# ChangUk/RecommenderSystems

Measured on AMD Instinct MI355X. Metric: RWR seeds/sec + achieved HBM GB/s on 100M-edge bipartite graph, 1/2/4/8 GPUs, higher is better.
Workload: dtype f64

## Files before the change

### include/rwr.h

```cpp
#ifndef RWR_H
#define RWR_H

#include <stdint.h>

#ifdef __cplusplus
extern "C" {
#endif

#define RWR_VERSION_STRING "0.4.0"

enum {
    RWR_OK            = 0,
    RWR_E_INVALID     = 1,
    RWR_E_RANGE       = 2,
    RWR_E_NO_DEVICE   = 3,
    RWR_E_HIP         = 4,
    RWR_E_NOMEM       = 5,
    RWR_E_CAPACITY    = 6,
    RWR_E_UNSUPPORTED = 7
};

enum { RWR_NODE_UNDEFINED = 0, RWR_NODE_USER = 1, RWR_NODE_ITEM = 2, RWR_NODE_ETC = 3 };
enum { RWR_EDGE_UNDEFINED = 0, RWR_EDGE_LIKE = 1, RWR_EDGE_FRIENDSHIP = 2, RWR_EDGE_FOLLOW = 3,
       RWR_EDGE_MENTION = 4, RWR_EDGE_AUTHORSHIP = 5, RWR_EDGE_PURCHASE = 6, RWR_EDGE_ETC = 7 };
// ... 12 lines not shown
    int32_t tile_group;
    int32_t profile;
    int64_t workspace_bytes;
    int32_t seed_row_kernel;
    int32_t reserved0;
} rwr_opts;

typedef struct rwr_stats {
    int32_t struct_size;
    int32_t n;
    int64_t nnz_raw;
    int64_t nnz;
    int32_t uniform;
    int32_t tile_seeds;
    int32_t tile_group;
    int32_t mode;
    double  build_ms;
    double  spmm_ms;
    int64_t spmm_launches;
    int64_t spmm_seed_steps;
    double  chain_ms;
    int64_t chain_launches;
    double  rank_ms;
    double  iterate_wall_ms;
    double  total_wall_ms;
    int64_t seeds_done;
    int64_t chain_redo_blocks;
    double  spmm_dense_ms;
    int64_t spmm_dense_launches;
    int64_t spmm_dense_seed_steps;
    int32_t uniform_path;
    int32_t reserved1;
    int64_t frontier_list_launches;
} rwr_stats;


const char *rwr_version(void);
int32_t rwr_device_count(void);
const char *rwr_last_error(void);

int32_t rwr_graph_create(int32_t n, const int64_t *node_id, const uint8_t *node_type,
                         const int64_t *rowptr , const int32_t *dst, const uint8_t *etype,
                         const double *w, const rwr_opts *opts , rwr_graph **out);
int32_t rwr_graph_destroy(rwr_graph *g);
int32_t rwr_graph_update_links(rwr_graph *g, int64_t count, const int64_t *link_index,
                               const uint8_t *etype , const double *w );
int32_t rwr_graph_append_links(rwr_graph *g, int64_t count, const int32_t *src, const int32_t *dst,
                               const uint8_t *etype, const double *w,
                               int64_t *new_index_out );
int32_t rwr_graph_size(const rwr_graph *g, int32_t *n, int64_t *nnz_raw, int64_t *nnz_explicit);
int32_t rwr_graph_get_normalized(rwr_graph *g, double *w_out , uint8_t *dangling_out );

int32_t rwr_recommend(rwr_graph *g, int32_t seed, float d, int32_t n_iter, int32_t top_n,
                      int64_t *out_id, double *out_score, int64_t *inout_count);

int32_t rwr_recommend_eval(rwr_graph *g, int32_t seed, float d, int32_t n_iter, const int64_t *test_ids,
                           int64_t n_test, int64_t *n_hits, double *sum_precision, int64_t *list_len);

int32_t rwr_recommend_eval_batch(rwr_graph *g, const int32_t *seeds, int32_t K, float d, int32_t n_iter,
                                 const int64_t *test_ptr, const int64_t *test_ids, int64_t *n_hits,
                                 double *sum_precision, int64_t *list_len);

typedef struct rwr_graph_desc {
    int32_t n_nodes;
    int32_t reserved0;
    const int64_t *node_id;
// ... 43 lines not shown
```

### recommendersystems_amd/_lib.py

```python
from __future__ import annotations

import ctypes as C
import os

_HERE = os.path.dirname(os.path.abspath(__file__))
LIB_PATH = os.path.join(_HERE, "librwr.so")

RWR_OK, RWR_E_INVALID, RWR_E_RANGE, RWR_E_NO_DEVICE, RWR_E_HIP, RWR_E_NOMEM, RWR_E_CAPACITY, RWR_E_UNSUPPORTED = range(8)
RWR_MODE_EXACT = 0
RWR_RUN_ITERATIONS, RWR_RUN_THRESHOLD, RWR_RUN_DEFAULT_THRESHOLD = 0, 1, 2

EXPORTS = [
    "rwr_version", "rwr_device_count", "rwr_last_error",
    "rwr_graph_create", "rwr_graph_update_links", "rwr_graph_append_links", "rwr_graph_destroy", "rwr_graph_size", "rwr_graph_get_normalized",
    "rwr_recommend", "rwr_recommend_eval", "rwr_recommend_eval_batch", "rwr_eval_graphs", "rwr_recommend_batch", "rwr_model_run", "rwr_model_deliver",
    "rwr_model_run_restart", "rwr_model_deliver_restart", "rwr_model_run_batch", "rwr_model_run_restart_batch",
    "rwr_part_begin", "rwr_part_step", "rwr_part_local_step", "rwr_part_finish_step", "rwr_part_rank",
    "rwr_get_stats", "rwr_reset_stats",
]


class rwr_opts(C.Structure):
    _fields_ = [("struct_size", C.c_int32), ("device", C.c_int32), ("mode", C.c_int32),
                ("tile_seeds", C.c_int32), ("tile_group", C.c_int32), ("profile", C.c_int32),
                ("workspace_bytes", C.c_int64), ("seed_row_kernel", C.c_int32), ("reserved0", C.c_int32)]


class rwr_graph_desc(C.Structure):
    _fields_ = [("n_nodes", C.c_int32), ("reserved0", C.c_int32), ("node_id", C.POINTER(C.c_int64)),
                ("node_type", C.POINTER(C.c_uint8)), ("rowptr", C.POINTER(C.c_int64)), ("dst", C.POINTER(C.c_int32)),
                ("etype", C.POINTER(C.c_uint8)), ("w", C.POINTER(C.c_double))]


class rwr_stats(C.Structure):
    _fields_ = [("struct_size", C.c_int32), ("n", C.c_int32), ("nnz_raw", C.c_int64), ("nnz", C.c_int64),
                ("uniform", C.c_int32), ("tile_seeds", C.c_int32), ("tile_group", C.c_int32), ("mode", C.c_int32),
                ("build_ms", C.c_double), ("spmm_ms", C.c_double), ("spmm_launches", C.c_int64),
                ("spmm_seed_steps", C.c_int64), ("chain_ms", C.c_double), ("chain_launches", C.c_int64),
                ("rank_ms", C.c_double), ("iterate_wall_ms", C.c_double), ("total_wall_ms", C.c_double),
                ("seeds_done", C.c_int64), ("chain_redo_blocks", C.c_int64),
                ("spmm_dense_ms", C.c_double), ("spmm_dense_launches", C.c_int64), ("spmm_dense_seed_steps", C.c_int64),
                ("uniform_path", C.c_int32), ("reserved1", C.c_int32), ("frontier_list_launches", C.c_int64)]


class RwrError(RuntimeError):
    def __init__(self, status: int, message: str):
        super().__init__(f"librwr status {status}: {message}")
        self.status = status


_lib = None


def load():
    global _lib
    if _lib is not None:
        return _lib
    if not os.path.exists(LIB_PATH):
        raise ImportError(f"{LIB_PATH} not found: build it with `python -c 'import __graft_entry__ as g; g.build()'` "
                          "(hipcc --offload-arch=gfx950); there is no CPU fallback")
    lib = C.CDLL(LIB_PATH)
    p = C.POINTER
    lib.rwr_version.restype = C.c_char_p
    lib.rwr_last_error.restype = C.c_char_p
    lib.rwr_device_count.restype = C.c_int32
    lib.rwr_graph_create.restype = C.c_int32
    lib.rwr_graph_create.argtypes = [C.c_int32, p(C.c_int64), p(C.c_uint8), p(C.c_int64), p(C.c_int32),
                                     p(C.c_uint8), p(C.c_double), p(rwr_opts), p(C.c_void_p)]
    lib.rwr_graph_update_links.restype = C.c_int32
    lib.rwr_graph_update_links.argtypes = [C.c_void_p, C.c_int64, p(C.c_int64), p(C.c_uint8), p(C.c_double)]
    lib.rwr_graph_append_links.restype = C.c_int32
    lib.rwr_graph_append_links.argtypes = [C.c_void_p, C.c_int64, p(C.c_int32), p(C.c_int32), p(C.c_uint8), p(C.c_double),
                                           p(C.c_int64)]
    lib.rwr_graph_destroy.restype = C.c_int32
    lib.rwr_graph_destroy.argtypes = [C.c_void_p]
# ... 58 lines not shown
```

### recommendersystems_amd/csrc/api.hip

```cpp
#include <stdarg.h>
#include <algorithm>
#include <cmath>
#include <mutex>
#include <vector>
#include <stdlib.h>
#include <string.h>

#include "engine.h"

namespace rwr {

static thread_local char g_err[512] = "";

void set_error(const char *fmt, ...)
{
    va_list ap;
    va_start(ap, fmt);
    vsnprintf(g_err, sizeof(g_err), fmt, ap);
    va_end(ap);
}

static int usable_devices()
{
    int n = 0;
// ... 896 lines not shown
    if (!g || !dev_y || !dev_r) { set_error("rwr_part_finish_step: NULL argument"); return RWR_E_INVALID; }
    RWR_BIND(g);
    return part_finish_step(g, (double *)dev_y, (const double *)dev_r);
}

int32_t rwr_part_rank(rwr_graph *g, void *dev_x, int32_t top_n, int64_t *ids, double *scores, int32_t *counts)
{
    g_err[0] = 0;
    if (!g || !dev_x || !ids || !scores || !counts) { set_error("rwr_part_rank: NULL argument"); return RWR_E_INVALID; }
    RWR_BIND(g);
    return part_rank(g, (double *)dev_x, top_n, ids, scores, counts);
}

int32_t rwr_get_stats(rwr_graph *g, rwr_stats *out)
{
    if (!g || !out) { set_error("rwr_get_stats: NULL argument"); return RWR_E_INVALID; }
    size_t sz = out->struct_size > 0 ? (size_t)out->struct_size : sizeof(rwr_stats);
    if (sz > sizeof(rwr_stats)) sz = sizeof(rwr_stats);
    rwr_stats s = g->stats;
    s.struct_size = (int32_t)sz;
    memcpy(out, &s, sz);
    return RWR_OK;
}

int32_t rwr_reset_stats(rwr_graph *g)
{
    if (!g) { set_error("rwr_reset_stats: NULL argument"); return RWR_E_INVALID; }
    rwr_stats &s = g->stats;
    s.spmm_ms = s.chain_ms = s.rank_ms = s.iterate_wall_ms = s.total_wall_ms = 0;
    s.spmm_launches = s.spmm_seed_steps = s.chain_launches = s.seeds_done = s.chain_redo_blocks = 0;
    s.spmm_dense_ms = 0;
    s.spmm_dense_launches = s.spmm_dense_seed_steps = 0;
    s.frontier_list_launches = 0;
    return RWR_OK;
}

}
```

### recommendersystems_amd/csrc/iterate.h

```cpp
#pragma once
#include "engine.h"
#include "step_plan.h"

namespace rwr {

struct SpmmArgs {
    const double *X = nullptr;
    double *Y = nullptr;
    const int32_t *seeds = nullptr;
    double c1 = 0.0;
    bool skip_seed_row = false;
    const uint32_t *nz_in = nullptr;
    uint32_t *nz_out = nullptr;
    const uint32_t *act = nullptr;
    const double *Zin = nullptr;
    double *Zout = nullptr;
    bool hub_scan = false;
    RowSource rows{};
};
void launch_spmm(rwr_graph *g, int G, int tg, const SpmmArgs &a, hipStream_t s);
void launch_init_seeds(rwr_graph *g, int G, int tg, double *X, const int32_t *seeds, uint32_t *nz, double *Z, double c1,
                       hipStream_t s);
void launch_make_z(int64_t elems, int G, const double *X, double *Z, const double *w_src, double c1, hipStream_t s);
void launch_make_z_nz(rwr_graph *g, int32_t lo, int32_t hi, int G, const double *X, double *Zs, double c1, uint32_t *nz,
// ... 1 lines not shown
void launch_mark_active(rwr_graph *g, int G, int tg, const uint32_t *nz, uint32_t *act, const int32_t *seeds, int32_t *fl_rows,
                        int32_t *fl_cnt, hipStream_t s);

struct Profile {
    const bool on;
    std::vector<hipEvent_t> pool, spmm, chain, rank, iter;
    size_t used = 0;
    std::vector<uint8_t> dense;
    explicit Profile(const rwr_graph *g) : on(g->opts.profile != 0) {}
    ~Profile() { for (auto e : pool) (void)hipEventDestroy(e); }
    int32_t record(hipEvent_t &e, hipStream_t s);
    int32_t end(std::vector<hipEvent_t> &stage, hipEvent_t a, hipStream_t s);
    void reset() { spmm.clear(); chain.clear(); rank.clear(); iter.clear(); dense.clear(); used = 0; }
    int32_t fold(rwr_graph *g);
};

struct GroupIter {
    rwr_graph *g;
    int G, tg;
    const int32_t *d_seeds;
    const int64_t *d_evoff;
    double c1;
    double *X, *Y;
    double *Zc = nullptr, *Zn = nullptr;
    uint32_t *nz_cur = nullptr, *nz_oth = nullptr;
    PlanConfig cfg;
    int64_t it = 0;
    int64_t dense_steps = 0;

    GroupIter(rwr_graph *g_, int G_, int tg_, const int32_t *seeds, const int64_t *evoff, double d)
        : g(g_), G(G_), tg(tg_), d_seeds(seeds), d_evoff(evoff), c1(1 - d) ,
          X(g_->X.p), Y(g_->Y.p), Zc(g_->vf ? g_->Z0.p : nullptr), Zn(g_->vf ? g_->Z1.p : nullptr) {}

    int32_t init(bool fresh = true, bool ranks_nonneg = true, bool ranking_only = false);
    int32_t step(const StepPlan &p, Profile &prof);
};

int32_t iterate_group(rwr_graph *g, int G, int tg, const int32_t *d_seeds, const int64_t *d_evoff, const int32_t *h_seeds,
                      double d, int64_t T, Profile &prof, double **final_X, int64_t *dense_steps);

int resolve_G(const rwr_graph *g, int32_t K);
int32_t ensure_workspace(rwr_graph *g, int G, int32_t K, int *TG_out, int extra_mats = 0);
int32_t upload_seed_slots(rwr_graph *g, const int32_t *seeds, int32_t K, int G, std::vector<int32_t> *slot_k_out,
                          std::vector<int32_t> *slot_seed_out = nullptr);

}
```

### recommendersystems_amd/csrc/iterate.hip

```cpp
#include "iterate.h"

#include <climits>
#include <cstdlib>
#include <type_traits>

namespace rwr {

template <int G, bool VF>
__global__ __launch_bounds__(256) void k_spmm(int32_t n, const int64_t *__restrict__ in_ptr,
                                              const int32_t *__restrict__ in_src,
                                              const double *__restrict__ in_w,
                                              const int32_t *__restrict__ row_order, int32_t nrows,
                                              const double *__restrict__ X, double *__restrict__ Y,
                                              const int32_t *__restrict__ seeds, double c1, int skip_seed_row,
                                              const double *__restrict__ w_src, double *__restrict__ Zout)
{
    constexpr int RPW = WAVE / G;
    constexpr int U = 4;
    const int tile = blockIdx.y;
    const size_t toff = (size_t)tile * (size_t)n * G;
    X += toff;
    Y += toff;
    if (VF && Zout) Zout += toff;
    const int lane = threadIdx.x & (WAVE - 1);
// ... 32 lines not shown
        }
        for (; p < e; ++p) {
            if (VF) {
                acc += X[(size_t)in_src[p] * G + k];
            } else {
                double rw = c1 * X[(size_t)in_src[p] * G + k];
                acc += rw * in_w[p];
            }
        }
        if (j >= 0 && j != my_seed) {
            Y[(size_t)j * G + k] = acc;
            if (VF && Zout) { const double rw = c1 * acc; Zout[(size_t)j * G + k] = rw * w_src[j]; }
        }
    }
}

template <int G, int CH, bool CHECK, bool WRITE, bool VF>
__device__ __forceinline__ void spmm_chunked_body(int32_t n, const int64_t *__restrict__ in_ptr,
                                                  const int32_t *__restrict__ in_src,
                                                  const double *__restrict__ in_w,
                                                  const int32_t *__restrict__ row_order, int32_t nrows,
                                                  const double *__restrict__ X, double *__restrict__ Y,
                                                  const int32_t *__restrict__ seeds, double c1,
                                                  int skip_seed_row, const uint32_t *__restrict__ nz_in,
                                                  uint32_t *__restrict__ nz_out,
                                                  const uint32_t *__restrict__ act,
                                                  const double *__restrict__ w_src, double *__restrict__ Zout)
{
    static_assert(G >= 8 && G <= 64, "chunked SpMM needs 8 <= G <= 64");
    constexpr int RPW = WAVE / G;
    const int tile = blockIdx.y;
    const size_t toff = (size_t)tile * (size_t)n * G;
    X += toff;
    Y += toff;
    if (VF && Zout) Zout += toff;
    const size_t nzw = ((size_t)n + 31) / 32;
    if (CHECK) nz_in += (size_t)tile * nzw;
    if (WRITE) nz_out += (size_t)tile * nzw;
    if (CHECK && act) act += (size_t)tile * nzw;
    const int lane = threadIdx.x & (WAVE - 1);
    const int sub = lane / G, k = lane % G;
    const int gbase = (lane - k) << 2;
    const int32_t my_seed = skip_seed_row ? seeds[tile * G + k] : -1;
    const int wpb = blockDim.x / WAVE;
    const int64_t nwaves = (int64_t)gridDim.x * wpb;
    for (int64_t rb = ((int64_t)blockIdx.x * wpb + threadIdx.x / WAVE) * RPW; rb < nrows; rb += nwaves * RPW) {
        const int64_t r = rb + sub;
        int32_t j = -1;
        int64_t p = 0, e = 0;
        if (r < nrows) {
            j = row_order[r];
            p = in_ptr[j];
            e = in_ptr[j + 1];
            if (CHECK && act && !((act[(uint32_t)j >> 5] >> (j & 31)) & 1u)) e = p;
        }
        double acc = 0.0;
        while (__any(p < e)) {
            const int64_t left = e - p;
            const int cnt = left > CH ? CH : (left > 0 ? (int)left : 0);
            int32_t my_idx = 0;
            double my_w = 0.0;
            if (k < cnt) {
                my_idx = in_src[p + k];
                if (!VF) my_w = in_w[p + k];
                if (CHECK) {
                    const uint32_t wd = nz_in[(uint32_t)my_idx >> 5];
                    if (!((wd >> (my_idx & 31)) & 1u)) my_idx |= (int32_t)0x80000000;
// ... 23 lines not shown
                                acc += rw * __hiloint2double(hi, lo);
                            }
                        }
                    }
                    p += cnt;
                    continue;
                }
            }
            double xv[CH], wv[CH];
#pragma unroll
            for (int t = 0; t < CH; ++t) {
                const int idx = __builtin_amdgcn_ds_bpermute(gbase + (t << 2), my_idx);
                if (!VF) {
                    const int lo = __builtin_amdgcn_ds_bpermute(gbase + (t << 2), wlo);
                    const int hi = __builtin_amdgcn_ds_bpermute(gbase + (t << 2), whi);
                    wv[t] = __hiloint2double(hi, lo);
                }
                xv[t] = (t < cnt && idx >= 0) ? X[(size_t)idx * G + k] : 0.0;
            }
#pragma unroll
            for (int t = 0; t < CH; ++t) {
                if (t < cnt) {
                    if (VF) {
                        acc += xv[t];
                    } else {
                        double rw = c1 * xv[t];
                        acc += rw * wv[t];
                    }
                }
            }
            p += cnt;
        }
        if (j >= 0 && j != my_seed) {
            Y[(size_t)j * G + k] = acc;
            if (VF && Zout) { const double rw = c1 * acc; Zout[(size_t)j * G + k] = rw * w_src[j]; }
        }
        if (WRITE) {
            const unsigned long long nzb = __ballot(acc != 0.0);
            const unsigned long long gmask = (G == 64) ? ~0ull : (((1ull << (G & 63)) - 1ull) << (sub * G));
            if (k == 0 && j >= 0 && (nzb & gmask)) atomicOr(&nz_out[(uint32_t)j >> 5], 1u << (j & 31));
        }
    }
}

template <int G, int CH, bool CHECK, bool WRITE, bool VF, bool LIST>
__global__ __launch_bounds__(256) void k_spmm_chunked(int32_t n, const int64_t *__restrict__ in_ptr,
                                                      const int32_t *__restrict__ in_src,
                                                      const double *__restrict__ in_w,
                                                      const int32_t *__restrict__ row_order, int32_t nrows,
                                                      const double *__restrict__ X, double *__restrict__ Y,
                                                      const int32_t *__restrict__ seeds, double c1,
                                                      int skip_seed_row, const uint32_t *__restrict__ nz_in,
                                                      uint32_t *__restrict__ nz_out,
                                                      const uint32_t *__restrict__ act,
                                                      const double *__restrict__ w_src, double *__restrict__ Zout)
{
    spmm_chunked_body<G, CH, CHECK, WRITE, VF>(n, in_ptr, in_src, in_w, row_order, nrows, X, Y, seeds, c1, skip_seed_row,
                                               nz_in, nz_out, act, w_src, Zout);
}

template <int G, int CH, bool VF>
__global__ __launch_bounds__(256) void k_spmm_frontier(int32_t n, const int64_t *__restrict__ in_ptr,
                                                       const int32_t *__restrict__ in_src,
                                                       const double *__restrict__ in_w,
                                                       const int32_t *__restrict__ fl_rows,
                                                       const int32_t *__restrict__ fl_cnt,
                                                       const double *__restrict__ X, double *__restrict__ Y,
// ... 185 lines not shown
    double acc = 0.0;
    for (size_t w0 = 0; w0 < nzw; w0 += WAVE) {
        const uint32_t word = (w0 + lane < nzw) ? bits[w0 + lane] : 0u;
        unsigned long long mask = __ballot(word != 0u);
        while (mask) {
            const int l = __builtin_ctzll(mask);
            mask &= mask - 1;
            uint32_t wv = (uint32_t)__builtin_amdgcn_readlane((int)word, l);
            while (wv) {
                const int b = __builtin_ctz(wv);
                wv &= wv - 1;
                const int32_t i = (int32_t)((w0 + l) * 32 + b);
                if (consumer && s >= 0) {
                    while (p < e && in_src[p] < i) ++p;
                    while (p < e && in_src[p] == i) { acc += termp[p]; ++p; }
                    const double xi = x[(size_t)i * G + k];
                    const double rw = c1 * xi;
                    acc += dangling[i] ? xi : (xi - rw);
                }
            }
        }
    }
    if (consumer && s >= 0) {
        Y[(size_t)tile * (size_t)n * G + (size_t)s * G + k] = acc;
        if (nz_out && acc != 0.0)
            atomicOr(&nz_out[(size_t)tile * nzw + ((uint32_t)s >> 5)], 1u << (s & 31));
    }
}

constexpr int CH3_NSW = 6;
constexpr int CH3_NST = CH3_NSW * WAVE;
constexpr int CH3_LPT = 16;
constexpr int CH3_CE = CH3_NST * CH3_LPT;
template <int G>
__global__ __launch_bounds__(WAVE + CH3_NST) void k_seed_chain_roles(
    int32_t n, const int64_t *__restrict__ in_ptr, const int32_t *__restrict__ in_src,
    const uint8_t *__restrict__ dangling, const double *__restrict__ X, double *__restrict__ Y,
    const int32_t *__restrict__ seeds, double c1, const int64_t *__restrict__ evoff,
    const double *__restrict__ evterm, uint32_t *__restrict__ nz_out, unsigned int *__restrict__ gate)
{
    if (threadIdx.x == 0 && gate) __hip_atomic_fetch_add(gate, 1u, __ATOMIC_RELAXED, __HIP_MEMORY_SCOPE_AGENT);
    constexpr int CR = CH3_CE / G;
    static_assert(CR % 32 == 0, "chunk rows must be a multiple of 32");
    extern __shared__ double rr[];
    const int tile = blockIdx.x;
    const double *x = X + (size_t)tile * (size_t)n * G;
    const int tid = threadIdx.x;
    const int64_t total = (int64_t)n * G;
    const int nchunks = (int)((total + CH3_CE - 1) / CH3_CE);

    if (tid >= WAVE) {
        const int st = tid - WAVE;
        double rega[CH3_LPT], regb[CH3_LPT];
        uint8_t dga[CH3_LPT], dgb[CH3_LPT];
#define CH3_LOAD(R, D, C)                                                       \
    {                                                                           \
        const int64_t base__ = (int64_t)(C) * CH3_CE;                           \
        _Pragma("unroll") for (int u = 0; u < CH3_LPT; ++u) {                   \
            int64_t el = base__ + (int64_t)u * CH3_NST + st;                    \
            el = el < total ? el : total - 1;                                   \
            R[u] = x[el];                                                       \
            D[u] = dangling[el / G];                                            \
        }                                                                       \
    }
#define CH3_STAGE(R, D, C)                                                                              \
    {                                                                                                   \
        const int64_t base__ = (int64_t)(C) * CH3_CE;                                                   \
        double *buf__ = rr + (size_t)((C) & 1) * CH3_CE;                                                \
        _Pragma("unroll") for (int u = 0; u < CH3_LPT; ++u) {                                           \
            const int off = u * CH3_NST + st;                                                           \
            const double xv = (base__ + off < total) ? R[u] : 0.0;   \
            const double rw = c1 * xv;                                                                  \
            buf__[off] = D[u] ? xv : (xv - rw);                                                         \
        }                                                                                               \
    }
        CH3_LOAD(rega, dga, 0)
        if (nchunks > 1) CH3_LOAD(regb, dgb, 1)
        for (int c = 0; c < nchunks; c += 2) {
            CH3_STAGE(rega, dga, c)
            if (c + 2 < nchunks) CH3_LOAD(rega, dga, c + 2)
            __builtin_amdgcn_fence(__ATOMIC_RELEASE, "workgroup", "local");
            __builtin_amdgcn_s_barrier();
            if (c + 1 < nchunks) {
                CH3_STAGE(regb, dgb, c + 1)
                if (c + 3 < nchunks) CH3_LOAD(regb, dgb, c + 3)
                __builtin_amdgcn_fence(__ATOMIC_RELEASE, "workgroup", "local");
                __builtin_amdgcn_s_barrier();
            }
        }
#undef CH3_LOAD
#undef CH3_STAGE
        return;
    }

    const bool consumer = tid < G;
    const int k = tid % G;
    int32_t s = -1;
    int64_t p = 0, e = 0;
    const int32_t *srcp = in_src;
    const double *termp = evterm;
    int32_t nxt = INT_MAX, raw_s = INT_MAX;
    double tcur = 0.0, raw_t = 0.0;
    bool has2 = false;
    if (consumer) {
        s = seeds[tile * G + k];
        if (s >= 0) {
            p = in_ptr[s];
            e = in_ptr[s + 1];
            termp = evterm + evoff[tile * G + k] - p;
            if (p < e) { nxt = srcp[p]; tcur = termp[p]; ++p; }
            if (p < e) { raw_s = srcp[p]; raw_t = termp[p]; has2 = true; ++p; }
        }
    }
    double acc = 0.0;
    __builtin_amdgcn_s_setprio(3);
    for (int c = 0; c < nchunks; ++c) {
        __builtin_amdgcn_s_barrier();
        __builtin_amdgcn_fence(__ATOMIC_ACQUIRE, "workgroup", "local");
// ... 91 lines not shown
    const int64_t j = ((int64_t)lo & ~(int64_t)63) + (int64_t)blockIdx.x * blockDim.x + threadIdx.x;
    bool any = false;
    if (j >= lo && j < hi) {
        const double w = w_src[j];
        const size_t at = (size_t)(j - lo) * G;
        for (int k = 0; k < G; ++k) {
            const double xv = X[(size_t)j * G + k];
            const double rw = c1 * xv;
            Zs[at + k] = rw * w;
            any = any || xv != 0.0;
        }
    }
    const unsigned long long m = __ballot(any);
    const int lane = threadIdx.x & (WAVE - 1);
    if (lane == 0 && (uint32_t)m) nz[(uint64_t)j >> 5] = (uint32_t)m;
    if (lane == 32 && (uint32_t)(m >> 32)) nz[(uint64_t)j >> 5] = (uint32_t)(m >> 32);
}


static PlanInput read_plan_knobs()
{
    PlanInput v;
    const char *e;
    if ((e = getenv("RWR_SPMM"))) v.spmm = atoi(e);
    if ((e = RWR_TUNE_ENV("RWR_NZ_ITERS"))) v.nz_iters = atoi(e);
    if ((e = getenv("RWR_ACT_ITERS"))) v.act_iters = atoi(e);
    if ((e = RWR_TUNE_ENV("RWR_ACT_MIN_N"))) v.act_min_n = atol(e);
    if ((e = getenv("RWR_FRONTIER_LIST"))) v.frontier_list = atoi(e);
    if ((e = getenv("RWR_CHAIN"))) v.chain = atoi(e);
    if ((e = RWR_TUNE_ENV("RWR_SCAN_WORK"))) v.scan_work = atof(e);
    if ((e = RWR_TUNE_ENV("RWR_SCAN_SIDE"))) v.scan_side = atoi(e);
    if ((e = RWR_TUNE_ENV("RWR_GATE"))) v.gate = atoi(e);
    if ((e = getenv("RWR_TAIL_ROWS"))) v.tail_rows = atoi(e);
    if ((e = RWR_TUNE_ENV("RWR_CHAIN_SERIAL"))) v.two_streams = atoi(e) == 0;
    return v;
}
static const PlanInput &plan_knobs() { static const PlanInput k = read_plan_knobs(); return k; }

template <class F> static void bool_dispatch(F &&f) { f(); }
template <class F, class... B> static void bool_dispatch(F &&f, bool b, B... bs)
{
    bool_dispatch([&](auto... c) { if (b) f(std::true_type{}, c...); else f(std::false_type{}, c...); }, bs...);
}

template <int G>
static void launch_spmm_g(rwr_graph *g, int tg, const SpmmArgs &a, hipStream_t s)
{
    const bool vf = a.Zin != nullptr;
    const double *GS = vf ? a.Zin : a.X;
    const int skip = a.skip_seed_row;
    constexpr int RPW = WAVE / G;
    constexpr int CH = G > 16 ? 16 : G;
    if constexpr (G >= 8) {
        if (a.rows.kind == Rows::Frontier) {
            const int32_t *fl_rows = g->fl_rows.p, *fl_cnt = g->fl_rows.p + (size_t)tg * (size_t)g->n;
            const unsigned want = cdiv((size_t)g->n / 10 + 1, (size_t)RPW * 4);
            const unsigned gx = want < 1u ? 1u : want < 2048u ? want : 2048u;
            bool_dispatch([&](auto v) {
                hipLaunchKernelGGL((k_spmm_frontier<G, CH, decltype(v)::value>), dim3(gx, tg), dim3(256), 0, s, g->n, g->in_ptr.p,
                                   g->in_src.p, g->in_w.p, fl_rows, fl_cnt, GS, a.Y, a.seeds, a.c1, skip, a.nz_in, a.nz_out,
                                   g->w_src.p, a.Zout);
            }, vf);
            return;
        }
    }
    const bool listed = a.rows.kind == Rows::Tail;
// ... 34 lines not shown
    hipLaunchKernelGGL(k_init_seeds, dim3(cdiv((size_t)tg * G, 64)), dim3(64), 0, s, g->n, tg, G, X, seeds, nz, Z, g->w_src.p, c1);
}
void launch_make_z(int64_t elems, int G, const double *X, double *Z, const double *w_src, double c1, hipStream_t s)
{
    hipLaunchKernelGGL(k_make_z, dim3(cdiv((size_t)elems, 256)), dim3(256), 0, s, elems, G, X, Z, w_src, c1);
}
void launch_make_z_nz(rwr_graph *g, int32_t lo, int32_t hi, int G, const double *X, double *Zs, double c1, uint32_t *nz,
                      hipStream_t s)
{
    const int64_t first = (int64_t)lo & ~(int64_t)63;
    hipLaunchKernelGGL(k_make_z_nz, dim3(cdiv((size_t)((int64_t)hi - first), 256)), dim3(256), 0, s, lo, hi, G, X, Zs, g->w_src.p,
                       c1, nz);
}
void launch_mark_active(rwr_graph *g, int G, int tg, const uint32_t *nz, uint32_t *act, const int32_t *seeds, int32_t *fl_rows,
                        int32_t *fl_cnt, hipStream_t s)
{
    const size_t nzw = ((size_t)g->n + 31) / 32;
    hipLaunchKernelGGL(k_mark_active, dim3(cdiv(nzw, 4), tg), dim3(256), 0, s, g->n, nz, act, g->rowptr.p, g->dst.p, g->etype.p,
                       G, seeds, fl_rows, fl_cnt);
}
template <int G>
static void launch_seed_terms(rwr_graph *g, int tg, const double *X, const int32_t *seeds, double c1,
                              const int64_t *evoff, hipStream_t s, const double *Zin, const uint32_t *nz = nullptr)
{
    const unsigned term_blocks = g->max_in_deg > 256 * 8 ? 8u : cdiv((size_t)(g->max_in_deg > 0 ? g->max_in_deg : 1), 256);
    bool_dispatch([&](auto v) {
        hipLaunchKernelGGL((k_seed_terms<G, decltype(v)::value>), dim3(term_blocks, tg * G), dim3(256), 0, s, g->n, g->in_ptr.p,
                           g->in_src.p, g->in_w.p, Zin ? Zin : X, seeds, c1, evoff, g->d_evterm.p, nz);
    }, Zin != nullptr);
}
template <int G>
static void launch_chain(rwr_graph *g, int tg, const double *X, double *Y, const int32_t *seeds, double c1,
                         const int64_t *evoff, uint32_t *nz_out, unsigned int *gate, hipStream_t s,
                         Chain kind, const uint32_t *nz_x)
{
    if (kind == Chain::Sparse) {
        hipLaunchKernelGGL(k_seed_chain_sparse<G>, dim3(tg), dim3(64), 0, s, g->n, g->in_ptr.p, g->in_src.p,
                           g->dangling.p, X, Y, seeds, c1, evoff, g->d_evterm.p, nz_x, nz_out, gate);
        return;
    }
    if (kind == Chain::Roles) {
        constexpr size_t smem = 2 * CH3_CE * sizeof(double);
        (void)hipFuncSetAttribute((const void *)k_seed_chain_roles<G>, hipFuncAttributeMaxDynamicSharedMemorySize, (int)smem);
        hipLaunchKernelGGL(k_seed_chain_roles<G>, dim3(tg), dim3(WAVE + CH3_NST), smem, s, g->n, g->in_ptr.p,
                           g->in_src.p, g->dangling.p, X, Y, seeds, c1, evoff, g->d_evterm.p, nz_out, gate);
        return;
    }
    hipLaunchKernelGGL(k_seed_chain<G>, dim3(cdiv((size_t)tg * G, 64)), dim3(64), 0, s, g->n, tg, g->in_ptr.p,
                       g->in_src.p, g->in_w.p, g->dangling.p, X, Y, seeds, c1, nz_out);
}

int32_t Profile::record(hipEvent_t &e, hipStream_t s)
{
    e = nullptr;
    if (!on) return RWR_OK;
    if (used == pool.size()) { RWR_HIP(hipEventCreate(&e)); pool.push_back(e); }
    e = pool[used++];
    RWR_HIP(hipEventRecord(e, s));
    return RWR_OK;
}
int32_t Profile::end(std::vector<hipEvent_t> &stage, hipEvent_t a, hipStream_t s)
{
    hipEvent_t b; RWR_TRY(record(b, s));
    if (on) stage.insert(stage.end(), {a, b});
    return RWR_OK;
}
int32_t Profile::fold(rwr_graph *g)
{
    auto drain = [&](const std::vector<hipEvent_t> &v, double *acc, bool dense_only) -> int32_t {
        for (size_t i = 0; i + 1 < v.size(); i += 2) {
            float ms = 0.f;
            if (dense_only && !dense[i / 2]) continue;
            RWR_HIP(hipEventElapsedTime(&ms, v[i], v[i + 1]));
            *acc += ms;
        }
        return RWR_OK;
    };
    if (on) {
        RWR_TRY(drain(spmm, &g->stats.spmm_dense_ms, true));
        RWR_TRY(drain(spmm, &g->stats.spmm_ms, false));
        RWR_TRY(drain(chain, &g->stats.chain_ms, false));
        RWR_TRY(drain(rank, &g->stats.rank_ms, false));
        RWR_TRY(drain(iter, &g->stats.iterate_wall_ms, false));
    }
    reset();
    return RWR_OK;
}

int32_t GroupIter::init(bool fresh, bool ranks_nonneg, bool ranking_only)
{
    const int32_t n = g->n;
    hipStream_t s = g->stream;
    const size_t elems = (size_t)tg * (size_t)n * G;
    PlanInput in = plan_knobs();
    in.n = n; in.nnz = g->nnz; in.nonneg = g->nonneg; in.big_n = spmv_big_n(); in.seed_row_kernel = g->opts.seed_row_kernel;
    in.scan_self = chain_scan_self_contained(G); in.G = G; in.tg = tg; in.c1 = c1;
    in.fresh = fresh; in.ranks_nonneg = ranks_nonneg; in.ranking_only = ranking_only;
    cfg = plan_config(in);
    if (fresh) RWR_HIP(hipMemsetAsync(X, 0, elems * sizeof(double), s));
    if (!fresh && Zc) launch_make_z((int64_t)elems, G, X, Zc, g->w_src.p, c1, s);
    const size_t nzw = ((size_t)n + 31) / 32;
    if (cfg.flist && g->fl_rows.ensure((size_t)tg * (size_t)n + (size_t)tg) != RWR_OK) {
        (void)hipGetLastError();
        cfg.flist = false;
    }
    if (fresh && Zc && !cfg.flist) RWR_HIP(hipMemsetAsync(Zc, 0, elems * sizeof(double), s));
    nz_cur = cfg.nz_iters > 0 ? g->d_nz.p : nullptr;
    nz_oth = cfg.nz_iters > 0 ? g->d_nz.p + (size_t)tg * nzw : nullptr;
    if (nz_cur) RWR_HIP(hipMemsetAsync(nz_cur, 0, (size_t)tg * nzw * sizeof(uint32_t), s));
    if (fresh) launch_init_seeds(g, G, tg, X, d_seeds, nz_cur, Zc, c1, s);
    RWR_HIP(hipGetLastError());
    if (cfg.scan) RWR_TRY(chain_scan_prepare(g, G, tg, d_seeds, s));
    if (Zc && G == 1 && tg == 1 && cfg.addends_nonneg) RWR_TRY(sweep_prepare(g));
    if (Zc && cfg.chain_kind == 0 && !cfg.scan) RWR_TRY(ensure_in_w(g));
    return RWR_OK;
}

int32_t GroupIter::step(const StepPlan &p, Profile &prof)
{
    const int32_t n = g->n;
    hipStream_t s = g->stream;
    const size_t nzw = ((size_t)n + 31) / 32;
    constexpr int GATE_SLOTS = 64;
    const uint32_t *nz_in = p.probe ? nz_cur : nullptr;
    uint32_t *nz_out = p.write_bits ? nz_oth : nullptr;
    if (nz_out) RWR_HIP(hipMemsetAsync(nz_out, 0, (size_t)tg * nzw * sizeof(uint32_t), s));
    uint32_t *act = p.mark ? g->d_nz.p + 2 * (size_t)tg * nzw : nullptr;
    const bool listed = p.rows.kind == Rows::Frontier;
    if (act) {
        int32_t *fl_rows = listed ? g->fl_rows.p : nullptr, *fl_cnt = listed ? fl_rows + (size_t)tg * (size_t)n : nullptr;
        RWR_HIP(hipMemsetAsync(act, 0, (size_t)tg * nzw * sizeof(uint32_t), s));
        if (fl_cnt) RWR_HIP(hipMemsetAsync(fl_cnt, 0, (size_t)tg * sizeof(int32_t), s));
        launch_mark_active(g, G, tg, nz_in, act, d_seeds, fl_rows, fl_cnt, s);
    }
    const uint32_t *nz_terms = p.terms_nz ? nz_in : nullptr;
    double *zout = (Zc && p.form_z) ? Zn : nullptr;
    hipStream_t sc = p.chain_side ? g->stream2 : s;
    unsigned int *gate_it = p.gate ? g->d_gate.p + (it % GATE_SLOTS) : nullptr;
    if (p.chain != Chain::None) {
        if (!p.scan()) RWR_DISPATCH_G(G, launch_seed_terms<GG>(g, tg, X, d_seeds, c1, d_evoff, s, Zc, nz_terms));
        if (gate_it) RWR_HIP(hipMemsetAsync(gate_it, 0, sizeof(unsigned int), s));
        if (p.chain_side) { RWR_HIP(hipEventRecord(g->ev_fork, s)); RWR_HIP(hipStreamWaitEvent(sc, g->ev_fork, 0)); }
        if (p.scan() && !(p.chain_self && Zc)) RWR_DISPATCH_G(G, launch_seed_terms<GG>(g, tg, X, d_seeds, c1, d_evoff, sc, Zc, nz_terms));
        hipEvent_t c0; RWR_TRY(prof.record(c0, sc));
        if (p.scan())
            RWR_TRY(chain_scan_step(g, G, tg, X, Y, d_seeds, d_evoff, c1, nz_out, sc, p.chain_self ? Zc : nullptr,
                                    p.chain_self ? zout : nullptr));
        else
            RWR_DISPATCH_G(G, launch_chain<GG>(g, tg, X, Y, d_seeds, c1, d_evoff, nz_out, gate_it, sc, p.chain, nz_in));
        RWR_TRY(prof.end(prof.chain, c0, sc));
        if (p.chain_side) RWR_HIP(hipEventRecord(g->ev_join, sc));
    }
    if (gate_it) hipLaunchKernelGGL(k_gate, dim3(1), dim3(1), 0, s, gate_it, (unsigned)(tg < 192 ? tg : 192));
    hipEvent_t a; RWR_TRY(prof.record(a, s));
    SpmmArgs sp;
    sp.X = X, sp.Y = Y, sp.seeds = d_seeds, sp.c1 = c1, sp.skip_seed_row = true;
    sp.nz_in = nz_in, sp.nz_out = nz_out, sp.act = act, sp.Zin = Zc, sp.Zout = zout;
    sp.hub_scan = cfg.addends_nonneg, sp.rows = p.rows;
    launch_spmm(g, G, tg, sp, s);
    RWR_TRY(prof.end(prof.spmm, a, s));
    if (prof.on) prof.dense.push_back(p.dense());
    if (p.dense()) { g->stats.spmm_dense_launches += 1; ++dense_steps; }
    if (p.chain_side) RWR_HIP(hipStreamWaitEvent(s, g->ev_join, 0));
    if (zout && p.seed_z) hipLaunchKernelGGL(k_seed_z, dim3(cdiv((size_t)tg * G, 64)), dim3(64), 0, s, n, tg, G, Y, zout, d_seeds, g->w_src.p, c1);
    RWR_HIP(hipGetLastError());
    { double *t = X; X = Y; Y = t; }
    { double *t = Zc; Zc = Zn; Zn = t; }
    { uint32_t *tz = nz_cur; nz_cur = nz_oth; nz_oth = tz; }
    g->stats.spmm_launches += 1;
    g->stats.chain_launches += p.chain != Chain::None; g->stats.frontier_list_launches += listed;
    ++it;
    return RWR_OK;
}

int32_t iterate_group(rwr_graph *g, int G, int tg, const int32_t *d_seeds, const int64_t *d_evoff, const int32_t *h_seeds,
                      double d, int64_t T, Profile &prof, double **final_X, int64_t *dense_steps)
{
    GroupIter gi(g, G, tg, d_seeds, d_evoff, d);
    RWR_TRY(gi.init(true, true, true));
    if (gi.cfg.tails) {
        RWR_TRY(tail_rows_prepare(g));
        gi.cfg.tail_depth = g->tail_depth;
        for (size_t q = 0; q < (size_t)tg * G; ++q)
            if (h_seeds[q] >= 0) gi.cfg.need |= g->h_tail_flag[h_seeds[q]];
    }
    while (gi.it < T) RWR_TRY(gi.step(plan_step(gi.cfg, gi.it, T), prof));
    *final_X = gi.X;
    *dense_steps = gi.dense_steps;
    return RWR_OK;
}

}
```

### recommendersystems_amd/csrc/step_plan.h

```cpp
#pragma once

#include <cstdint>

namespace rwr {

struct PlanInput {
    int spmm = 1, nz_iters = 4, act_iters = -1, frontier_list = 1, chain = 1;
    int64_t act_min_n = 200000; double scan_work = 10000.0;
    int scan_side = 1, gate = 1, tail_rows = 1;
    bool two_streams = true;
    int32_t n = 0, big_n = 2000000;
    int64_t nnz = 0; bool nonneg = true;
    int seed_row_kernel = 0;
    bool scan_self = false;
    int G = 1, tg = 1;
    double c1 = 0.85;
    bool fresh = true;
    bool ranks_nonneg = true;
    bool ranking_only = false;
};

struct PlanConfig {
    int G = 1, tg = 1; bool fresh = true;
    int nz_iters = 0;
    int act_iters = 0;
    bool flist = false;
    bool addends_nonneg = false;
    bool scan = false;
    int chain_kind = 1;
    bool scan_side = false, scan_self = false;
    bool two_streams = true, gate = true;
    bool tails = false; int tail_depth = 0;
    unsigned need = 0;
};

inline PlanConfig plan_config(const PlanInput &in)
{
    PlanConfig c;
    c.G = in.G, c.tg = in.tg, c.fresh = in.fresh;
    const bool single = in.G == 1 && in.tg == 1;
    c.nz_iters = (in.G >= 8 && in.spmm != 0 && in.nonneg) ? in.nz_iters : 0;
    c.act_iters = in.act_iters >= 0 ? in.act_iters : ((in.nnz / (in.n > 0 ? in.n : 1)) <= 64 ? 2 : 1);
    if (single && in.act_iters < 0 && c.act_iters == 2 && in.n >= in.big_n) c.act_iters = 3;
    if (single && in.spmm != 0 && in.nonneg) c.nz_iters = c.act_iters;
    if (single && in.act_iters < 0 && in.n < in.act_min_n) c.nz_iters = c.act_iters = 0;
    if (!in.fresh) c.nz_iters = c.act_iters = 0;
    c.flist = in.ranking_only && in.fresh && in.frontier_list != 0 && in.G >= 8 && c.nz_iters >= 2 && c.act_iters >= 1;
    c.chain_kind = in.seed_row_kernel == 1 ? 3 : in.seed_row_kernel == 2 ? 2 : in.seed_row_kernel == 3 ? 0 : in.chain;
    const double per_seed = 0.89 * (double)in.nnz / (double)(in.n > 0 ? in.n : 1) + 6.7;
    c.addends_nonneg = in.c1 >= 0.0 && in.c1 <= 1.0 && in.nonneg && in.ranks_nonneg;
    c.scan = c.addends_nonneg && (c.chain_kind == 2 || (c.chain_kind == 1 && (double)in.tg * in.G * per_seed < in.scan_work));
    c.scan_side = in.scan_side != 0 && single && in.two_streams && in.n >= 100000;
    c.scan_self = in.scan_self, c.two_streams = in.two_streams, c.gate = in.gate != 0;
    c.tails = in.ranking_only && in.tail_rows != 0 && !single;
    return c;
}

enum class Rows : uint8_t { All, Frontier, Tail };
struct RowSource { Rows kind = Rows::All; int level = 0; };
enum class Chain : uint8_t { None, Scan, ScanSide, Sparse, Roles, Simple };

struct StepPlan {
    RowSource rows;
    bool probe = false, write_bits = false;
    bool mark = false;
    bool terms_nz = false;
    Chain chain = Chain::None;
    bool chain_side = false, gate = false;
    bool chain_self = false;
    bool form_z = false, seed_z = false;
    bool dense() const { return !probe && rows.kind == Rows::All; }
    bool scan() const { return chain == Chain::Scan || chain == Chain::ScanSide; }
};

inline int last_tail(const PlanConfig &c)
{
    for (int k = 0; c.tails && k < c.tail_depth; ++k)
        if ((c.need >> k) & 1u) return k;
    return c.tails ? c.tail_depth - 1 : -1;
}

inline StepPlan plan_step(const PlanConfig &c, int64_t it, int64_t T)
{
    StepPlan p;
    const int64_t k = T - 1 - it;
    const bool last = T >= 0 && k == 0, tail = T >= 0 && k <= last_tail(c);
    p.probe = it < c.nz_iters;
    p.write_bits = it + 1 < c.nz_iters;
    p.mark = p.probe && it < c.act_iters;
    p.terms_nz = c.flist && p.probe;
    if (tail)
        p.rows = {Rows::Tail, (int)k};
    else if (c.flist && T >= 0 && !last && p.mark && p.write_bits && (it + 1 < c.act_iters || it == 1))
        p.rows = {Rows::Frontier, 0};
    if (tail && !((c.need >> k) & 1u)) p.chain = Chain::None;
    else if (c.scan && (!p.mark || c.G == 1)) p.chain = c.scan_side ? Chain::ScanSide : Chain::Scan;
    else if (p.mark) p.chain = Chain::Sparse;
    else p.chain = c.chain_kind == 0 ? Chain::Simple : Chain::Roles;
    const bool fold = p.chain != Chain::None && !p.scan();
    p.chain_side = p.chain == Chain::ScanSide || (fold && c.two_streams);
    p.gate = fold && c.two_streams && c.gate;
    p.chain_self = p.scan() && c.scan_self;
    p.form_z = !last;
    p.seed_z = p.form_z && p.chain != Chain::None && !p.chain_self;
    return p;
}

}
```

Measured before the change: 762.3.

## Skip dead X stores in SpMM and probe-gate chain loads via nz bitmap

```diff
diff --git a/include/rwr.h b/include/rwr.h
--- a/include/rwr.h
+++ b/include/rwr.h
@@ -68,6 +68,8 @@
     int32_t uniform_path;
     int32_t reserved1;
     int64_t frontier_list_launches;
+    int64_t spmm_x_stores_skipped;
+    int64_t chain_probe_launches;
 } rwr_stats;
 
 
diff --git a/recommendersystems_amd/_lib.py b/recommendersystems_amd/_lib.py
--- a/recommendersystems_amd/_lib.py
+++ b/recommendersystems_amd/_lib.py
@@ -40,7 +40,8 @@
                 ("rank_ms", C.c_double), ("iterate_wall_ms", C.c_double), ("total_wall_ms", C.c_double),
                 ("seeds_done", C.c_int64), ("chain_redo_blocks", C.c_int64),
                 ("spmm_dense_ms", C.c_double), ("spmm_dense_launches", C.c_int64), ("spmm_dense_seed_steps", C.c_int64),
-                ("uniform_path", C.c_int32), ("reserved1", C.c_int32), ("frontier_list_launches", C.c_int64)]
+                ("uniform_path", C.c_int32), ("reserved1", C.c_int32), ("frontier_list_launches", C.c_int64),
+                ("spmm_x_stores_skipped", C.c_int64), ("chain_probe_launches", C.c_int64)]
 
 
 class RwrError(RuntimeError):
diff --git a/recommendersystems_amd/csrc/api.hip b/recommendersystems_amd/csrc/api.hip
--- a/recommendersystems_amd/csrc/api.hip
+++ b/recommendersystems_amd/csrc/api.hip
@@ -952,7 +952,8 @@
     s.spmm_dense_ms = 0;
     s.spmm_dense_launches = s.spmm_dense_seed_steps = 0;
     s.frontier_list_launches = 0;
-    return RWR_OK;
-}
-
-}
+    s.spmm_x_stores_skipped = s.chain_probe_launches = 0;
+    return RWR_OK;
+}
+
+}
diff --git a/recommendersystems_amd/csrc/iterate.h b/recommendersystems_amd/csrc/iterate.h
--- a/recommendersystems_amd/csrc/iterate.h
+++ b/recommendersystems_amd/csrc/iterate.h
@@ -57,7 +57,8 @@
         : g(g_), G(G_), tg(tg_), d_seeds(seeds), d_evoff(evoff), c1(1 - d) ,
           X(g_->X.p), Y(g_->Y.p), Zc(g_->vf ? g_->Z0.p : nullptr), Zn(g_->vf ? g_->Z1.p : nullptr) {}
 
-    int32_t init(bool fresh = true, bool ranks_nonneg = true, bool ranking_only = false);
+    int32_t init(bool fresh = true, bool ranks_nonneg = true, bool ranking_only = false, int64_t T = -1,
+                 const int32_t *h_seeds = nullptr);
     int32_t step(const StepPlan &p, Profile &prof);
 };
 
diff --git a/recommendersystems_amd/csrc/iterate.hip b/recommendersystems_amd/csrc/iterate.hip
--- a/recommendersystems_amd/csrc/iterate.hip
+++ b/recommendersystems_amd/csrc/iterate.hip
@@ -88,7 +88,8 @@
     const int tile = blockIdx.y;
     const size_t toff = (size_t)tile * (size_t)n * G;
     X += toff;
-    Y += toff;
+    const bool store_x = Y != nullptr;
+    if (store_x) Y += toff;
     if (VF && Zout) Zout += toff;
     const size_t nzw = ((size_t)n + 31) / 32;
     if (CHECK) nz_in += (size_t)tile * nzw;
@@ -178,7 +179,7 @@
             p += cnt;
         }
         if (j >= 0 && j != my_seed) {
-            Y[(size_t)j * G + k] = acc;
+            if (store_x) Y[(size_t)j * G + k] = acc;
             if (VF && Zout) { const double rw = c1 * acc; Zout[(size_t)j * G + k] = rw * w_src[j]; }
         }
         if (WRITE) {
@@ -430,12 +431,13 @@
 constexpr int CH3_NST = CH3_NSW * WAVE;
 constexpr int CH3_LPT = 16;
 constexpr int CH3_CE = CH3_NST * CH3_LPT;
-template <int G>
+template <int G, bool PROBE>
 __global__ __launch_bounds__(WAVE + CH3_NST) void k_seed_chain_roles(
     int32_t n, const int64_t *__restrict__ in_ptr, const int32_t *__restrict__ in_src,
     const uint8_t *__restrict__ dangling, const double *__restrict__ X, double *__restrict__ Y,
     const int32_t *__restrict__ seeds, double c1, const int64_t *__restrict__ evoff,
-    const double *__restrict__ evterm, uint32_t *__restrict__ nz_out, unsigned int *__restrict__ gate)
+    const double *__restrict__ evterm, uint32_t *__restrict__ nz_out, unsigned int *__restrict__ gate,
+    const uint32_t *__restrict__ nz_x)
 {
     if (threadIdx.x == 0 && gate) __hip_atomic_fetch_add(gate, 1u, __ATOMIC_RELAXED, __HIP_MEMORY_SCOPE_AGENT);
     constexpr int CR = CH3_CE / G;
@@ -451,37 +453,53 @@
         const int st = tid - WAVE;
         double rega[CH3_LPT], regb[CH3_LPT];
         uint8_t dga[CH3_LPT], dgb[CH3_LPT];
-#define CH3_LOAD(R, D, C)                                                       \
+        const uint32_t *bits = PROBE ? nz_x + (size_t)tile * (((size_t)n + 31) / 32) : nullptr;
+        uint32_t lva = 0xffffu, lvb = 0xffffu;
+#define CH3_LOAD(R, D, LV, C)                                                   \
     {                                                                           \
         const int64_t base__ = (int64_t)(C) * CH3_CE;                           \
+        if (PROBE) {                                                            \
+            uint32_t live__ = 0u;                                               \
+            _Pragma("unroll") for (int u = 0; u < CH3_LPT; ++u) {               \
+                int64_t r0 = (base__ + (int64_t)u * CH3_NST + (st & ~(WAVE - 1))) / G; \
+                r0 = r0 < n ? r0 : n - 1;                                       \
+                const uint32_t wd = bits[__builtin_amdgcn_readfirstlane((int)(r0 >> 5))]; \
+                int64_t el = base__ + (int64_t)u * CH3_NST + st;                \
+                el = el < total ? el : total - 1;                               \
+                live__ |= ((wd >> ((uint32_t)(el / G) & 31u)) & 1u) << u;       \
+            }                                                                   \
+            LV = live__;                                                        \
+        }                                                                       \
         _Pragma("unroll") for (int u = 0; u < CH3_LPT; ++u) {                   \
             int64_t el = base__ + (int64_t)u * CH3_NST + st;                    \
             el = el < total ? el : total - 1;                                   \
+            if (PROBE) el = ((LV >> u) & 1u) ? el : 0;                          \
             R[u] = x[el];                                                       \
             D[u] = dangling[el / G];                                            \
         }                                                                       \
     }
-#define CH3_STAGE(R, D, C)                                                                              \
+#define CH3_STAGE(R, D, LV, C)                                                                          \
     {                                                                                                   \
         const int64_t base__ = (int64_t)(C) * CH3_CE;                                                   \
         double *buf__ = rr + (size_t)((C) & 1) * CH3_CE;                                                \
         _Pragma("unroll") for (int u = 0; u < CH3_LPT; ++u) {                                           \
             const int off = u * CH3_NST + st;                                                           \
-            const double xv = (base__ + off < total) ? R[u] : 0.0;   \
+                                \
+            const double xv = (base__ + off < total && (!PROBE || ((LV >> u) & 1u))) ? R[u] : 0.0;      \
             const double rw = c1 * xv;                                                                  \
             buf__[off] = D[u] ? xv : (xv - rw);                                                         \
         }                                                                                               \
     }
-        CH3_LOAD(rega, dga, 0)
-        if (nchunks > 1) CH3_LOAD(regb, dgb, 1)
+        CH3_LOAD(rega, dga, lva, 0)
+        if (nchunks > 1) CH3_LOAD(regb, dgb, lvb, 1)
         for (int c = 0; c < nchunks; c += 2) {
-            CH3_STAGE(rega, dga, c)
-            if (c + 2 < nchunks) CH3_LOAD(rega, dga, c + 2)
+            CH3_STAGE(rega, dga, lva, c)
+            if (c + 2 < nchunks) CH3_LOAD(rega, dga, lva, c + 2)
             __builtin_amdgcn_fence(__ATOMIC_RELEASE, "workgroup", "local");
             __builtin_amdgcn_s_barrier();
             if (c + 1 < nchunks) {
-                CH3_STAGE(regb, dgb, c + 1)
-                if (c + 3 < nchunks) CH3_LOAD(regb, dgb, c + 3)
+                CH3_STAGE(regb, dgb, lvb, c + 1)
+                if (c + 3 < nchunks) CH3_LOAD(regb, dgb, lvb, c + 3)
                 __builtin_amdgcn_fence(__ATOMIC_RELEASE, "workgroup", "local");
                 __builtin_amdgcn_s_barrier();
             }
@@ -639,6 +657,8 @@
     if ((e = RWR_TUNE_ENV("RWR_SCAN_SIDE"))) v.scan_side = atoi(e);
     if ((e = RWR_TUNE_ENV("RWR_GATE"))) v.gate = atoi(e);
     if ((e = getenv("RWR_TAIL_ROWS"))) v.tail_rows = atoi(e);
+    if ((e = getenv("RWR_DEAD_STORES"))) v.dead_stores = atoi(e);
+    if ((e = getenv("RWR_CHAIN_PROBE"))) v.chain_probe = atoi(e);
     if ((e = RWR_TUNE_ENV("RWR_CHAIN_SERIAL"))) v.two_streams = atoi(e) == 0;
     return v;
 }
@@ -739,7 +759,7 @@
 template <int G>
 static void launch_chain(rwr_graph *g, int tg, const double *X, double *Y, const int32_t *seeds, double c1,
                          const int64_t *evoff, uint32_t *nz_out, unsigned int *gate, hipStream_t s,
-                         Chain kind, const uint32_t *nz_x)
+                         Chain kind, const uint32_t *nz_x, bool probe)
 {
     if (kind == Chain::Sparse) {
         hipLaunchKernelGGL(k_seed_chain_sparse<G>, dim3(tg), dim3(64), 0, s, g->n, g->in_ptr.p, g->in_src.p,
@@ -748,9 +768,12 @@
     }
     if (kind == Chain::Roles) {
         constexpr size_t smem = 2 * CH3_CE * sizeof(double);
-        (void)hipFuncSetAttribute((const void *)k_seed_chain_roles<G>, hipFuncAttributeMaxDynamicSharedMemorySize, (int)smem);
-        hipLaunchKernelGGL(k_seed_chain_roles<G>, dim3(tg), dim3(WAVE + CH3_NST), smem, s, g->n, g->in_ptr.p,
-                           g->in_src.p, g->dangling.p, X, Y, seeds, c1, evoff, g->d_evterm.p, nz_out, gate);
+        bool_dispatch([&](auto pr) {
+            const auto kern = k_seed_chain_roles<G, decltype(pr)::value>;
+            (void)hipFuncSetAttribute((const void *)kern, hipFuncAttributeMaxDynamicSharedMemorySize, (int)smem);
+            hipLaunchKernelGGL(kern, dim3(tg), dim3(WAVE + CH3_NST), smem, s, g->n, g->in_ptr.p, g->in_src.p, g->dangling.p, X, Y,
+                               seeds, c1, evoff, g->d_evterm.p, nz_out, gate, nz_x);
+        }, probe && nz_x != nullptr);
         return;
     }
     hipLaunchKernelGGL(k_seed_chain<G>, dim3(cdiv((size_t)tg * G, 64)), dim3(64), 0, s, g->n, tg, g->in_ptr.p,
@@ -794,7 +817,7 @@
     return RWR_OK;
 }
 
-int32_t GroupIter::init(bool fresh, bool ranks_nonneg, bool ranking_only)
+int32_t GroupIter::init(bool fresh, bool ranks_nonneg, bool ranking_only, int64_t T, const int32_t *h_seeds)
 {
     const int32_t n = g->n;
     hipStream_t s = g->stream;
@@ -802,15 +825,21 @@
     PlanInput in = plan_knobs();
     in.n = n; in.nnz = g->nnz; in.nonneg = g->nonneg; in.big_n = spmv_big_n(); in.seed_row_kernel = g->opts.seed_row_kernel;
     in.scan_self = chain_scan_self_contained(G); in.G = G; in.tg = tg; in.c1 = c1;
-    in.fresh = fresh; in.ranks_nonneg = ranks_nonneg; in.ranking_only = ranking_only;
+    in.fresh = fresh; in.ranks_nonneg = ranks_nonneg; in.ranking_only = ranking_only; in.vf = Zc != nullptr;
     cfg = plan_config(in);
-    if (fresh) RWR_HIP(hipMemsetAsync(X, 0, elems * sizeof(double), s));
-    if (!fresh && Zc) launch_make_z((int64_t)elems, G, X, Zc, g->w_src.p, c1, s);
-    const size_t nzw = ((size_t)n + 31) / 32;
     if (cfg.flist && g->fl_rows.ensure((size_t)tg * (size_t)n + (size_t)tg) != RWR_OK) {
         (void)hipGetLastError();
         cfg.flist = false;
     }
+    if (cfg.tails && h_seeds) {
+        RWR_TRY(tail_rows_prepare(g));
+        cfg.tail_depth = g->tail_depth;
+        for (size_t q = 0; q < (size_t)tg * G; ++q)
+            if (h_seeds[q] >= 0) cfg.need |= g->h_tail_flag[h_seeds[q]];
+    }
+    if (fresh && plan_clear_x(cfg, T)) RWR_HIP(hipMemsetAsync(X, 0, elems * sizeof(double), s));
+    if (!fresh && Zc) launch_make_z((int64_t)elems, G, X, Zc, g->w_src.p, c1, s);
+    const size_t nzw = ((size_t)n + 31) / 32;
     if (fresh && Zc && !cfg.flist) RWR_HIP(hipMemsetAsync(Zc, 0, elems * sizeof(double), s));
     nz_cur = cfg.nz_iters > 0 ? g->d_nz.p : nullptr;
     nz_oth = cfg.nz_iters > 0 ? g->d_nz.p + (size_t)tg * nzw : nullptr;
@@ -854,14 +883,14 @@
             RWR_TRY(chain_scan_step(g, G, tg, X, Y, d_seeds, d_evoff, c1, nz_out, sc, p.chain_self ? Zc : nullptr,
                                     p.chain_self ? zout : nullptr));
         else
-            RWR_DISPATCH_G(G, launch_chain<GG>(g, tg, X, Y, d_seeds, c1, d_evoff, nz_out, gate_it, sc, p.chain, nz_in));
+            RWR_DISPATCH_G(G, launch_chain<GG>(g, tg, X, Y, d_seeds, c1, d_evoff, nz_out, gate_it, sc, p.chain, nz_in, p.chain_probe));
         RWR_TRY(prof.end(prof.chain, c0, sc));
         if (p.chain_side) RWR_HIP(hipEventRecord(g->ev_join, sc));
     }
     if (gate_it) hipLaunchKernelGGL(k_gate, dim3(1), dim3(1), 0, s, gate_it, (unsigned)(tg < 192 ? tg : 192));
     hipEvent_t a; RWR_TRY(prof.record(a, s));
     SpmmArgs sp;
-    sp.X = X, sp.Y = Y, sp.seeds = d_seeds, sp.c1 = c1, sp.skip_seed_row = true;
+    sp.X = X, sp.Y = p.store_x ? Y : nullptr, sp.seeds = d_seeds, sp.c1 = c1, sp.skip_seed_row = true;
     sp.nz_in = nz_in, sp.nz_out = nz_out, sp.act = act, sp.Zin = Zc, sp.Zout = zout;
     sp.hub_scan = cfg.addends_nonneg, sp.rows = p.rows;
     launch_spmm(g, G, tg, sp, s);
@@ -876,6 +905,7 @@
     { uint32_t *tz = nz_cur; nz_cur = nz_oth; nz_oth = tz; }
     g->stats.spmm_launches += 1;
     g->stats.chain_launches += p.chain != Chain::None; g->stats.frontier_list_launches += listed;
+    g->stats.spmm_x_stores_skipped += !p.store_x; g->stats.chain_probe_launches += p.chain_probe;
     ++it;
     return RWR_OK;
 }
@@ -884,13 +914,7 @@
                       double d, int64_t T, Profile &prof, double **final_X, int64_t *dense_steps)
 {
     GroupIter gi(g, G, tg, d_seeds, d_evoff, d);
-    RWR_TRY(gi.init(true, true, true));
-    if (gi.cfg.tails) {
-        RWR_TRY(tail_rows_prepare(g));
-        gi.cfg.tail_depth = g->tail_depth;
-        for (size_t q = 0; q < (size_t)tg * G; ++q)
-            if (h_seeds[q] >= 0) gi.cfg.need |= g->h_tail_flag[h_seeds[q]];
-    }
+    RWR_TRY(gi.init(true, true, true, T, h_seeds));
     while (gi.it < T) RWR_TRY(gi.step(plan_step(gi.cfg, gi.it, T), prof));
     *final_X = gi.X;
     *dense_steps = gi.dense_steps;
diff --git a/recommendersystems_amd/csrc/step_plan.h b/recommendersystems_amd/csrc/step_plan.h
--- a/recommendersystems_amd/csrc/step_plan.h
+++ b/recommendersystems_amd/csrc/step_plan.h
@@ -6,6 +6,7 @@
 
 struct PlanInput {
     int spmm = 1, nz_iters = 4, act_iters = -1, frontier_list = 1, chain = 1;
+    int dead_stores = 1, chain_probe = 1;
     int64_t act_min_n = 200000; double scan_work = 10000.0;
     int scan_side = 1, gate = 1, tail_rows = 1;
     bool two_streams = true;
@@ -18,6 +19,7 @@
     bool fresh = true;
     bool ranks_nonneg = true;
     bool ranking_only = false;
+    bool vf = false;
 };
 
 struct PlanConfig {
@@ -32,6 +34,8 @@
     bool two_streams = true, gate = true;
     bool tails = false; int tail_depth = 0;
     unsigned need = 0;
+    bool dead_stores = false;
+    bool chain_probe = false;
 };
 
 inline PlanConfig plan_config(const PlanInput &in)
@@ -53,6 +57,8 @@
     c.scan_side = in.scan_side != 0 && single && in.two_streams && in.n >= 100000;
     c.scan_self = in.scan_self, c.two_streams = in.two_streams, c.gate = in.gate != 0;
     c.tails = in.ranking_only && in.tail_rows != 0 && !single;
+    c.dead_stores = in.dead_stores != 0 && in.ranking_only && in.vf && in.G >= 8 && in.spmm != 0;
+    c.chain_probe = in.chain_probe != 0 && c.flist && c.addends_nonneg;
     return c;
 }
 
@@ -69,6 +75,8 @@
     bool chain_side = false, gate = false;
     bool chain_self = false;
     bool form_z = false, seed_z = false;
+    bool store_x = true;
+    bool chain_probe = false;
     bool dense() const { return !probe && rows.kind == Rows::All; }
     bool scan() const { return chain == Chain::Scan || chain == Chain::ScanSide; }
 };
@@ -80,7 +88,7 @@
     return c.tails ? c.tail_depth - 1 : -1;
 }
 
-inline StepPlan plan_step(const PlanConfig &c, int64_t it, int64_t T)
+inline StepPlan plan_step_own(const PlanConfig &c, int64_t it, int64_t T)
 {
     StepPlan p;
     const int64_t k = T - 1 - it;
@@ -106,4 +114,27 @@
     return p;
 }
 
+inline bool reads_x(const StepPlan &next) { return next.chain != Chain::None; }
+inline bool reads_through_bitmap(const StepPlan &p)
+{
+    return p.probe && p.terms_nz && (p.chain == Chain::None || p.chain == Chain::Sparse || (p.chain == Chain::Roles && p.chain_probe));
 }
+
+inline StepPlan plan_step(const PlanConfig &c, int64_t it, int64_t T)
+{
+    StepPlan p = plan_step_own(c, it, T);
+    if (c.dead_stores && T >= 0 && it + 1 < T) p.store_x = reads_x(plan_step_own(c, it + 1, T));
+    p.chain_probe = c.chain_probe && c.flist && p.probe && p.chain == Chain::Roles && it >= 1 &&
+                    plan_step_own(c, it - 1, T).rows.kind == Rows::Frontier;
+    return p;
+}
+
+inline bool plan_clear_x(const PlanConfig &c, int64_t T)
+{
+    if (!c.chain_probe || !c.flist || T < 3) return true;
+    const StepPlan p0 = plan_step(c, 0, T), p1 = plan_step(c, 1, T), p2 = plan_step(c, 2, T);
+    if (p1.rows.kind != Rows::Frontier) return true;
+    return !(reads_through_bitmap(p0) && reads_through_bitmap(p2));
+}
+
+}
```

Result: no change. 767.0 (median of 6 runs) (+0.6%).
